# tatsuya-ogawa/GaussianSplattingMlx

Hardware: AMD Instinct MI355X
Metric: train views/sec (full step: fwd + L1/DSSIM loss + bwd + Adam + densify/prune at the reference cadence), Lego 800x800 300k Gaussians (higher is better)
Workload: dtype f32

## Files before the change

gaussiansplattingmlx_amd/_lib.py:

```python
from __future__ import annotations

import ctypes as C
import os

HERE = os.path.dirname(os.path.abspath(__file__))
LIB_PATH = os.environ.get("GSPLAT_LIB", os.path.join(HERE, "libgsplat_hip.so"))

GS_OK = 0
STATUS = {1: "GS_ERR_INVALID_ARG", 2: "GS_ERR_SIZE_MISMATCH", 3: "GS_ERR_WORKSPACE_OVERFLOW", 4: "GS_ERR_HIP",
          5: "GS_ERR_NO_FORWARD", 6: "GS_ERR_NO_DEVICE", 7: "GS_ERR_IO", 8: "GS_ERR_COMM", 9: "GS_ERR_REPLICA_MISMATCH"}
GS_ERR_REPLICA_MISMATCH = 9


class GsplatError(RuntimeError):
    def __init__(self, code, msg):
        super().__init__(f"{STATUS.get(code, code)}: {msg}")
        self.code = code


class gs_camera(C.Structure):
    _fields_ = [("view", C.c_float * 16), ("proj", C.c_float * 16), ("cam_center", C.c_float * 3),
                ("fov_x", C.c_float), ("fov_y", C.c_float), ("focal_x", C.c_float), ("focal_y", C.c_float)]


# ... 88 lines not shown
    "gs_ply_pack_rows": (C.c_int, [_vp, C.c_int, C.c_int] + [_vp] * 7),
    "gs_set_block_work_buffer": (C.c_int, [_vp, _vp]),
    "gs_view_hint_words": (C.c_int, [_vp, C.POINTER(C.c_int)]),
    "gs_set_view_hints": (C.c_int, [_vp, _vp, C.c_int]),
    "gs_set_depth_cuts": (C.c_int, [_vp, C.c_int]),
    "gs_clear_depth_cuts": (C.c_int, [_vp, _vp, C.c_int]),
    "gs_forward_missed": (C.c_int, [_vp, C.POINTER(C.c_int)]),
    "gs_cut_stats": (C.c_int, [_vp, C.POINTER(C.c_uint32)]),
    "gs_set_grad_norm_accum": (C.c_int, [_vp, _vp]),
    "gs_block_count": (C.c_int, [_vp, _vp]),
    "gs_copy_block_work": (C.c_int, [_vp, _vp]),
    "gs_dist_topk": (C.c_int, [_vp, C.c_int, C.c_int, C.c_int, C.c_int, _vp, _vp]),
    "gs_sh_grad_from_views_adam": (C.c_int, [_vp, C.c_int, C.c_int, C.c_int] + [_vp] * 8 + [C.c_longlong] + [C.c_float] * 6),
    "gs_loss_target_cache_floats": (C.c_int, [_vp, C.POINTER(C.c_longlong)]),
    "gs_set_loss_target_cache": (C.c_int, [_vp, _vp, C.c_int]),
    "gs_set_loss_mask": (C.c_int, [_vp, _vp]),
    "gs_loss_forward_backward": (C.c_int, [_vp] + [_vp] * 5 + [C.c_float, C.c_float] + [_vp] * 3),
    "gs_depth_loss": (C.c_int, [_vp, C.POINTER(gs_depth_loss_params)] + [_vp] * 7),
    "gs_depth_normalize": (C.c_int, [_vp, C.c_longlong, _vp, _vp, C.c_float, _vp]),
    "gs_adam_step": (C.c_int, [_vp, C.c_longlong] + [_vp] * 4 + [C.c_int, _vp, _vp] + [C.c_float] * 4),
    "gs_profile_enable": (C.c_int, [_vp, C.c_uint]),
    "gs_profile_read": (C.c_int, [_vp, _vp, _vp]),
    "gs_copy_last_contrib": (C.c_int, [_vp, _vp]),
    "gs_last_stats": (C.c_int, [_vp, C.POINTER(C.c_uint32)]),
    "gs_ctx_set_tuning": (C.c_int, [_vp, C.c_int, C.c_longlong]),
    "gs_copy_overflow_flag": (C.c_int, [_vp, _vp]),
    "gs_set_update_gate": (C.c_int, [_vp, _vp]),
    "gs_set_overflow_rider": (C.c_int, [_vp, _vp]),
    "gs_set_pose_correction": (C.c_int, [_vp, _vp, _vp]),
    "gs_set_exposure": (C.c_int, [_vp, _vp, _vp]),
    "gs_apply_exposure": (C.c_int, [_vp, C.c_longlong, _vp, _vp, _vp]),
    "gs_set_bilateral_grid": (C.c_int, [_vp, _vp, _vp, C.c_int, C.c_int, C.c_int, C.c_float]),
    "gs_apply_bilateral_grid": (C.c_int, [_vp, C.c_int, C.c_int, _vp, C.c_int, C.c_int, C.c_int, _vp, _vp]),
    "gs_set_antialiasing": (C.c_int, [_vp, C.c_int]),
    "gs_set_background": (C.c_int, [_vp, _vp]),
    "gs_get_background": (C.c_int, [_vp, _vp]),
    "gs_composite_target": (C.c_int, [_vp, C.c_longlong, _vp, _vp, _vp, _vp]),
    "gs_set_absgrad": (C.c_int, [_vp, C.c_int]),
    "gs_get_absgrad": (C.c_int, [_vp, C.c_int, _vp]),
    "gs_set_sparse_adam": (C.c_int, [_vp, C.c_int]),
    "gs_get_visibility": (C.c_int, [_vp, C.c_int, _vp]),
    "gs_adam_step_visible": (C.c_int, [_vp, C.c_longlong] + [_vp] * 4 + [C.c_int, _vp, _vp, _vp] + [C.c_float] * 4 + [C.c_int, _vp]),
    "gs_set_filter3d_cameras": (C.c_int, [_vp, C.c_int, _vp]),
    "gs_compute_filter3d": (C.c_int, [_vp, C.c_int, _vp, _vp]),
    "gs_set_filter3d": (C.c_int, [_vp, _vp]),
    "gs_filter3d_bake": (C.c_int, [_vp, C.c_int] + [_vp] * 5),
# ... 14 lines not shown

_lib = None


def load():
    global _lib
    if _lib is not None:
        return _lib
    if not os.path.exists(LIB_PATH):
        raise ImportError(f"{LIB_PATH} is missing: run `python -m gaussiansplattingmlx_amd.build` "
                          "(or __graft_entry__.build()). There is no CPU fallback.")
    import torch
    lib = C.CDLL(LIB_PATH)
    for name, (res, args) in _SIGS.items():
        fn = getattr(lib, name)
        fn.restype = res
        fn.argtypes = args
    _lib = lib
    return lib


TUNE_FWD_WAVES_PER_SIMD, TUNE_BWD_WAVES_PER_CU, TUNE_FWD_QUADRANTS, TUNE_OP_FWD_PPL, TUNE_OP_BWD_PPL, \
    TUNE_FWD_TRACE_BUFFER, TUNE_DEPTH_GRADIENT, TUNE_WIDE_TILE_SORT, TUNE_HOST_OVERFLOW_ERRORS, TUNE_SPLITTER_DEPTH_SORT, \
    TUNE_COLOUR_RIDERS, TUNE_FWD_QUEUES, TUNE_FWD_FOUR_WAVES, TUNE_FWD_FOLD_TEST_SCALE, TUNE_POISON_CHECKPOINTS, TUNE_RENDER_ONLY, TUNE_FWD_PAIR, TUNE_FWD_SLOW_SLOT, TUNE_TRIM_RECTS = range(19)


def exported_symbols():
    return list(_SIGS)


def make_camera(view, proj, camCenter, fovX, fovY, focalX, focalY) -> gs_camera:
    import numpy as np
    cam = gs_camera()
    v = np.asarray(view, dtype=np.float32).reshape(16)
    p = np.asarray(proj, dtype=np.float32).reshape(16)
    cc = np.asarray(camCenter, dtype=np.float32).reshape(3)
    for i in range(16):
        cam.view[i] = float(v[i])
        cam.proj[i] = float(p[i])
    for i in range(3):
        cam.cam_center[i] = float(cc[i])
    cam.fov_x, cam.fov_y, cam.focal_x, cam.focal_y = float(fovX), float(fovY), float(focalX), float(focalY)
    return cam
```

gaussiansplattingmlx_amd/csrc/api.hip:

```cpp
#include <math.h>
#include <stdlib.h>
#include <stdio.h>
#include <string.h>

#include "gs_ctx.h"
#include <vector>

using namespace gs;

namespace {

int fail(gs_ctx* c, int code, const std::string& msg)
{
    if (c) c->err = msg;
    return code;
}

template <class T>
int dev_alloc(gs_ctx* c, T** p, size_t count)
{
    *p = nullptr;
    if (count == 0) count = 1;
    GS_HIP_CHECK(c, hipMalloc((void**)p, count * sizeof(T)));
    c->ws_bytes += count * sizeof(T);
// ... 820 lines not shown
    if (c->fwd.cutsActive && !c->fwd.missChecked) GS_HIP_CHECK(c, hipEventSynchronize(c->fwdDone));
    c->fwd.missed = false;
    c->fwd.bwdPrepared = false;
    c->fwd.arenaOverflow = false;
    c->fwd.cutStore = c->cutStore;
    c->fwd.cutsActive = c->cutStore != nullptr && c->allowCuts && N > 0;
    c->fwd.missChecked = !c->fwd.cutsActive;
    if (c->fwd.cutsActive) c->missHost[0] = 0;
    const CamParams cp = make_cam(cam, c->W, c->H);
    if (c->poseDelta) {
        const long long need = pose_partials_floats(N);
        if (need > c->posePartialsCap) {
            GS_HIP_CHECK(c, hipStreamSynchronize(c->stream));
            dev_free(c->posePartials);
            c->posePartialsCap = 0;
            if (const int arc = dev_alloc(c, &c->posePartials, (size_t)need)) return arc;
            c->posePartialsCap = need;
        }
        if (const int prc = launch_pose_camera(c, cp, c->poseDelta)) return prc;
    }
    c->segBaseWanted = c->fast16 && N > 0;
    c->segBaseDone = false;
    c->fwdPairNow = c->fast16 && blend_forward_v2_pair_decide(c);
    int rc = bin_with_capacity(c, N, reserved, !c->fast16, [&]() {
        return launch_projection_fused_forward(c, N, K, xyz, features_dc, features_rest, scales, rotation, opacity, cp,
                                               radii);
    });
    c->segBaseWanted = false;
    if (rc) { c->rider.on = false; return rc; }
    if (c->rider.on && c->rider.next < c->rider.total) {
        GsStageTimer t(c, GS_STAGE_PROJ_FWD, true);
        if ((rc = launch_colour_rest(c))) return rc;
    }
    c->rider.on = false;
    {
        GsStageTimer t(c, GS_STAGE_BLEND_FWD);
        rc = c->fast16 ? launch_blend_forward_v2(c, out_color, out_depth, out_alpha)
                       : launch_blend_forward(c, c->bg, out_color, out_depth, out_alpha, c->lastContrib);
        if (rc) return rc;
    }
    if (c->fwd.cutsActive) GS_HIP_CHECK(c, hipEventRecord(c->fwdDone, c->stream));
    c->fwd.valid = true;
    c->absgradN = -1;
    c->fwd.blendBackwardDone = false;
    c->fwd.consumed = false;
    c->fwd.blockWork = c->blockWork;
// ... 689 lines not shown
    case GS_TUNE_WIDE_TILE_SORT:
        c->wideTileSort = value != 0; return GS_OK;
    case GS_TUNE_DEPTH_GRADIENT:
        c->depthGradient = value != 0; return GS_OK;
    case GS_TUNE_HOST_OVERFLOW_ERRORS:
        c->hostOverflowErrors = value != 0; return GS_OK;
    case GS_TUNE_SPLITTER_DEPTH_SORT:
        c->splitterSort = value < 0 ? 0 : (value > 2 ? 2 : (int)value); c->haveSplitters = false; return GS_OK;
    case GS_TUNE_COLOUR_RIDERS:
        c->colourRiders = (int)value; return GS_OK;
    case GS_TUNE_FWD_FOLD_TEST_SCALE:
        if (value < 1 || value > 1000) return fail(c, GS_ERR_INVALID_ARG, "gs_ctx_set_tuning: fold test scale is in permille, 1..1000");
        c->fwdFoldScale = (float)value / 1000.0f; return GS_OK;
    case GS_TUNE_POISON_CHECKPOINTS:
        c->poisonCheckpoints = value != 0; return GS_OK;
    case GS_TUNE_RENDER_ONLY:
        c->renderOnly = value != 0; return GS_OK;
    case GS_TUNE_FWD_SLOW_SLOT:
        if (value < 1 || value > 16) return fail(c, GS_ERR_INVALID_ARG, "gs_ctx_set_tuning: the first slow wave slot must be 1..16 (16 = none)");
        c->fwdSlowSlot = (int)value; return GS_OK;
    case GS_TUNE_FWD_PAIR:
        if (value < -1 || value > 16) return fail(c, GS_ERR_INVALID_ARG, "gs_ctx_set_tuning: forward pair workgroups per CU must be -1 (by list depth), 0..16");
        c->fwdPair = (int)value; return GS_OK;
    case GS_TUNE_TRIM_RECTS:
        if (value < 0 || value > 2) return fail(c, GS_ERR_INVALID_ARG, "gs_ctx_set_tuning: trim rects is 0 (the reference's squares), 1 (cut by the ellipse's box) or 2 (and into four row groups)");
        c->trimRects = value != 0; c->rowGroups = value == 2; return GS_OK;
    case GS_TUNE_FWD_TRACE_BUFFER:
        c->fwdTrace = reinterpret_cast<unsigned long long*>((uintptr_t)value); return GS_OK;
    default:
        return fail(c, GS_ERR_INVALID_ARG, "gs_ctx_set_tuning: unknown knob");
    }
}

int gs_copy_overflow_flag(gs_ctx* c, uint32_t* out)
{
    if (!c || !out) return GS_ERR_INVALID_ARG;
    hipLaunchKernelGGL(copy_word_kernel, dim3(1), dim3(1), 0, c->stream, c->counters + GS_CNT_OVERFLOW, out);
    GS_HIP_CHECK(c, hipGetLastError());
    return GS_OK;
}

int gs_set_update_gate(gs_ctx* c, const uint32_t* gate)
{
    if (!c) return GS_ERR_INVALID_ARG;
    c->adamGate = gate ? gate : c->counters + GS_CNT_OVERFLOW;
    return GS_OK;
// ... 34 lines not shown
int gs_block_count(gs_ctx* c, int* n)
{
    if (!c || !n) return GS_ERR_INVALID_ARG;
    *n = c->numPixBlocks;
    return GS_OK;
}

int gs_copy_block_work(gs_ctx* c, uint32_t* out)
{
    if (!c || !out) return GS_ERR_INVALID_ARG;
    if (!c->fwd.valid) return fail(c, GS_ERR_NO_FORWARD, "gs_copy_block_work: no gs_render_forward on this context");
    if (!c->fast16) return fail(c, GS_ERR_INVALID_ARG, "gs_copy_block_work: only for tile sizes served by the fused kernels");
    GS_HIP_CHECK(c, hipMemcpyAsync(out, c->fwd.blockWork, sizeof(uint32_t) * (size_t)c->numPixBlocks, hipMemcpyDeviceToDevice,
                                   c->stream));
    return GS_OK;
}

int gs_copy_last_contrib(gs_ctx* c, uint32_t* out)
{
    if (!c || !out) return GS_ERR_INVALID_ARG;
    if (!c->fwd.valid) return fail(c, GS_ERR_NO_FORWARD, "gs_copy_last_contrib: no gs_render_forward on this context");
    GS_HIP_CHECK(c, hipMemcpyAsync(out, c->lastContrib, sizeof(uint32_t) * (size_t)c->W * c->H, hipMemcpyDeviceToDevice,
                                   c->stream));
    return GS_OK;
}

int gs_adam_step(gs_ctx* c, long long n, float* params, const float* grads, float* m, float* v, int nseg,
                 const long long* seg_end, const float* seg_lr, float beta1, float beta2, float eps, float grad_scale)
{
    if (!c) return GS_ERR_INVALID_ARG;
    if (n < 0 || nseg < 1 || nseg > 8 || !seg_end || !seg_lr) return fail(c, GS_ERR_INVALID_ARG, "gs_adam_step: bad segments");
    if (n > 0 && (!params || !grads || !m || !v)) return fail(c, GS_ERR_INVALID_ARG, "gs_adam_step: null buffer");
    if (((uintptr_t)params | (uintptr_t)grads | (uintptr_t)m | (uintptr_t)v) & 15)
        return fail(c, GS_ERR_INVALID_ARG, "gs_adam_step: arenas must be 16-byte aligned");
    long long prev = 0;
    for (int i = 0; i < nseg; i++) {
        if (seg_end[i] < prev || seg_end[i] > n) return fail(c, GS_ERR_INVALID_ARG, "gs_adam_step: segments not ascending");
        prev = seg_end[i];
    }
    if (prev != n) return fail(c, GS_ERR_SIZE_MISMATCH, "gs_adam_step: segments do not cover the arena");
    { const int orc = deferred_overflow(c); if (orc) return orc; }
    return launch_adam(c, n, params, grads, m, v, nseg, seg_end, seg_lr, beta1, beta2, eps, grad_scale);
}

int gs_adam_step_visible(gs_ctx* c, long long n, float* params, const float* grads, float* m, float* v, int nseg,
                         const long long* seg_end, const float* seg_lr, const int* seg_row_floats, float beta1, float beta2,
// ... 266 lines not shown
```

gaussiansplattingmlx_amd/csrc/blend_v2.hip:

```cpp
#include "gs_ctx.h"
#include "gs_bwd_prep.h"
#include "gs_cull.h"
#include "gs_wavesum.h"

namespace gs {

constexpr int BLK = 16;
constexpr uint32_t CKPT_POOL_MAX = 8;
static inline uint32_t ckpt_pool(uint32_t partSlots, uint32_t waves)
{
    const uint32_t perWave = partSlots / (waves / 8u + 1u);
    return perWave >= CKPT_POOL_MAX ? CKPT_POOL_MAX : (perWave < 1u ? 1u : perWave);
}

struct Rec {
    float mx, my, c00, c01, c10, c11, r, g, b, op, depth;
};

#ifndef GS_FWD_PREFETCH
#define GS_FWD_PREFETCH 1
#endif

typedef float f4 __attribute__((ext_vector_type(4)));
typedef float f2 __attribute__((ext_vector_type(2)));
// ... 488 lines not shown

        V2P_BARRIER();
        for (uint32_t c0 = 0; c0 < count; c0 += 64) {
            const uint32_t cur = (c0 >> 6) & 1u;
            const f4* sl = sg[cur];
            const uint32_t n = __builtin_amdgcn_readfirstlane(*(volatile uint32_t*)&sN[cur]);
            br += cr; bgr += cg; bb += cb; cr = 0.f; cg = 0.f; cb = 0.f;
            if (DEPTH) { bd += dd; dd = 0.f; }
            if (statePlanes != 0 && c0 != 0 && (c0 % SEG) == 0) save_state(c0);
            bool live = true;
            for (uint32_t j = 0; j < n; j += 4) {
                Pre p0, p1, p2, p3;
                pre(sl, j, p0); pre(sl, j + 1, p1); pre(sl, j + 2, p2); pre(sl, j + 3, p3);
                post(p0); post(p1); post(p2); post(p3);
                if (!any_live()) { live = false; break; }
            }
            if (live) {
                if (T >= 1e-4f) nc = min(c0 + 64u, count);
                live = any_live();
            }
            if (!live && lane == 0) sStop = 1u;
            V2P_BARRIER();
            if (*(volatile uint32_t*)&sStop) break;
        }
        V2P_BARRIER();
        if (bRaw != 0xFFFFFFFFu) {
            if (cutStore && any_live() && lane == 0 && cutStore[tile] != 0u) hostWords[0] = 1u;
            if (in) {
                const size_t pix = (size_t)y * W + x;
                float bg0, bg1, bg2;
                gs_bg_terms(bgc, T, bg0, bg1, bg2);
                outColor[3 * pix] = (br + cr) + bg0; outColor[3 * pix + 1] = (bgr + cg) + bg1; outColor[3 * pix + 2] = (bb + cb) + bg2;
                if (DEPTH) outDepth[pix] = bd + dd;
                outAlpha[pix] = 1.0f - T; lastContrib[pix] = nc; finalT[pix] = T;
            }
            uint32_t m = in ? nc : 0u;
#pragma unroll
            for (int d = 32; d >= 1; d >>= 1) m = max(m, (uint32_t)__shfl_xor((int)m, d, 64));
            if (lane == 0 && m) atomicMax(&blockWork[b], m);
        }
    }
}
#undef V2P_BARRIER

#define GS_V2W_WGS 5
template <int SEG, bool DEPTH>
// ... 504 lines not shown
                const uint32_t src = (0x6a4b98331ull >> ((q - 2) * 4)) & 15u;
                v = (DEPTH || q != 10) ? part[j][src] : 0.0f;
                if (q < 6) v *= -0.5f;
            }
            if (v != 0.0f) atomicAdd(&gradAcc16[(size_t)(idx[i0 + j] & idxMask) * 16 + (ABSGRAD && q >= 11 ? q + 1 : q)], v);
        }
        __builtin_amdgcn_s_waitcnt(0xc07f);
        __builtin_amdgcn_wave_barrier();
    }
}

constexpr int SEGLEN = GS_SEG_LEN;
bool blend_forward_v2_wide(const gs_ctx* c)
{
    if (c->fwdTrace || !c->fwdQuadrants) return false;
    return c->fwdWide == 1 || (c->fwdWide < 0 && c->numPixBlocks * 4 <= c->numCUs * 4 * c->fwdWavesPerSimd);
}
bool blend_forward_v2_pair_decide(const gs_ctx* c)
{
    if (c->fwdTrace || !c->fwdQuadrants || blend_forward_v2_wide(c)) return false;
    if (c->fwdPair >= 0) return c->fwdPair != 0;
    const unsigned long long lastM = c->missHost ? c->missHost[8] : 0u;
    return c->numPixBlocks > 0 && lastM / (unsigned long long)c->numPixBlocks >= 4500ull;
}
bool blend_forward_v2_pair(const gs_ctx* c)
{
    return c->fwdPairNow;
}
int blend_forward_v2_grid(const gs_ctx* c)
{
    const int fwdItems = c->numPixBlocks * 4;
    const int fwdGrid = blend_forward_v2_wide(c) ? c->numCUs * GS_V2W_WGS
                        : blend_forward_v2_pair(c) ? c->numCUs * (c->fwdPair > 1 ? c->fwdPair : GS_V2P_WGS)
                                                   : c->numCUs * 4 * c->fwdWavesPerSimd;
    return fwdGrid > fwdItems ? fwdItems : fwdGrid;
}

void fill_seg_base(gs_ctx* c, SegBaseArgs& a)
{
    a.nBlocks = c->numPixBlocks; a.blocksX = c->blocksX; a.tileW = c->tileW; a.tileH = c->tileH; a.gridW = c->gridW;
    a.tileRanges = c->tileRanges; a.tileTotal = nullptr;
    a.segBase = c->segBase; a.blockWork = c->blockWork; a.counters = c->counters; a.workHint = c->workHint;
    a.blockOrder = c->blockOrder; a.queueStart = (uint32_t)blend_forward_v2_grid(c); a.fwdQueue = c->fwdQueue; a.nq = c->fwdQueues; a.spatial = c->fwdSpatial;
}

int launch_blend_forward_v2(gs_ctx* c, float* outColor, float* outDepth, float* outAlpha)
// ... 23 lines not shown
        c->fwd.qslotStatic = ownW * (uint32_t)grid * 4u;
        const uint32_t partW = (qcap - c->fwd.qslotStatic) / 8u;
        auto kw = outDepth ? blend_fwd_v2w_kernel<SEGLEN, true> : blend_fwd_v2w_kernel<SEGLEN, false>;
        hipLaunchKernelGGL(kw, dim3(grid), dim3(256), 0, c->stream, c->W, c->H, c->tileW,
                           c->tileH, c->gridW, blocksX, nItems, c->bg, reinterpret_cast<const float4*>(c->packed12),
                           c->sortedRaw, c->idxMask, c->tileRanges, c->segBase, (uint32_t)c->segCap, c->renderOnly ? 0 : c->fwd.statePlanes, outColor, outDepth,
                           outAlpha, c->lastContrib, c->finalT, c->segState, c->segSlot, qcap, ownW, partW, ckpt_pool(partW, (uint32_t)grid * 4u), c->blockWork, c->counters, c->fwdQueue,
                           (uint32_t)c->fwdQueues, c->blockOrder, cuts, c->missDev, c->fwdFoldScale, c->virt);
        GS_HIP_CHECK(c, hipGetLastError());
        if (c->renderOnly) c->fwd.statePlanes = 0;
        return GS_OK;
    }
    if (blend_forward_v2_pair(c)) {
        auto kp = outDepth ? blend_fwd_v2p_kernel<SEGLEN, true> : blend_fwd_v2p_kernel<SEGLEN, false>;
        hipLaunchKernelGGL(kp, dim3(grid), dim3(128), 0, c->stream, c->W, c->H, c->tileW,
                           c->tileH, c->gridW, blocksX, nItems, c->bg, reinterpret_cast<const float4*>(c->packed12),
                           c->sortedRaw, c->idxMask, c->tileRanges, c->segBase, (uint32_t)c->segCap, c->renderOnly ? 0 : c->fwd.statePlanes, outColor, outDepth,
                           outAlpha, c->lastContrib, c->finalT, c->segState, c->segSlot, qcap, own, partSlots, ckpt_pool(partSlots, (uint32_t)grid), c->blockWork, c->counters, c->fwdQueue, (uint32_t)c->fwdQueues, c->blockOrder,
                           cuts, c->missDev, c->virt);
        GS_HIP_CHECK(c, hipGetLastError());
        if (c->renderOnly) c->fwd.statePlanes = 0;
        return GS_OK;
    }
    auto kern = outDepth ? blend_fwd_v2q_kernel<SEGLEN, true> : blend_fwd_v2q_kernel<SEGLEN, false>;
    hipLaunchKernelGGL(kern, dim3(grid / 4), dim3(256), 0, c->stream, c->W, c->H, c->tileW,
                       c->tileH, c->gridW, blocksX, nItems, c->bg, reinterpret_cast<const float4*>(c->packed12),
                       c->sortedRaw, c->idxMask, c->tileRanges, c->segBase, (uint32_t)c->segCap, c->renderOnly ? 0 : c->fwd.statePlanes, outColor, outDepth,
                       outAlpha, c->lastContrib, c->finalT, c->segState, c->segSlot, qcap, own, partSlots, ckpt_pool(partSlots, (uint32_t)grid), c->blockWork, c->counters, c->fwdQueue, (uint32_t)c->fwdQueues, c->blockOrder,
                       c->fwdTrace, cuts, c->missDev, (uint32_t)c->fwdSlowSlot, c->virt);
    GS_HIP_CHECK(c, hipGetLastError());
    if (c->renderOnly) c->fwd.statePlanes = 0;
    return GS_OK;
}

void fill_bwd_prep(gs_ctx* c, int N, uint32_t queueStart, BwdPrepArgs& p)
{
    p.nBlocks = c->numPixBlocks;
    p.blockWork = c->fwd.blockWork;
    p.itemBlock = c->itemBlock;
    p.itemRow = c->itemRow;
    p.segBase = c->segBase;
    p.itemCap = (uint32_t)c->itemCap;
    p.counters = c->counters;
    p.queueStart = queueStart;
    p.bwdQueue = c->bwdQueue;
    p.clearBuf = reinterpret_cast<float4*>(c->gradAcc16);
// ... 43 lines not shown
```

gaussiansplattingmlx_amd/csrc/gs_ctx.h:

```cpp
#pragma once
#include <hip/hip_runtime.h>
#include <stdint.h>

#include <string>
#include <vector>

#include "../../include/gsplat.h"
#include "gs_math.h"

enum {
    GS_CNT_M = 0,
    GS_CNT_OVERFLOW = 1,
    GS_CNT_MREQ = 2,
    GS_CNT_B = 3,
    GS_CNT_NVIS = 4,
    GS_CNT_CONTRIB_LO = 5,
    GS_CNT_CONTRIB_HI = 6,
    GS_CNT_ITEMS = 9,
    GS_CNT_QUEUE = 10,
    GS_CNT_QUEUE_FWD = 11,
    GS_CNT_CUT_DROPPED = 12,
    GS_CNT_QSLOTS = 16,
    GS_CNT_COUNT = 24
};
// ... 60 lines not shown
struct GsVirtGeom {
    int nbx = 0, nby = 0;
    int tw = 0, th = 0;
};
__device__ __forceinline__ void gs_block_pixels(const GsVirtGeom& g, int bx, int by, int W, int H, int& X0, int& Y0, int& XL, int& YL)
{
    if (g.nbx == 0) { X0 = bx * 16; Y0 = by * 16; XL = W; YL = H; return; }
    const int tx = bx / g.nbx, ix = bx - tx * g.nbx, ty = by / g.nby, iy = by - ty * g.nby;
    X0 = tx * g.tw + ix * 16; Y0 = ty * g.th + iy * 16;
    XL = min(W, min(X0 + 16, (tx + 1) * g.tw)); YL = min(H, min(Y0 + 16, (ty + 1) * g.th));
}
constexpr int GS_F3D_CAM_FLOATS = 16;
constexpr int GS_CUT_SUPER = 4;
struct GsCutCoarse {
    const uint32_t* superCut = nullptr;
    int superW = 0;
    uint32_t* dropPerBlock = nullptr;
};
struct GsRealGeom {
    int tileW = 16, tileH = 16, gridW = 0, gridH = 0, T = 0, tileBits = 1;
    bool fast16 = false;
};

struct gs_ctx {
    int device = 0;
    GsDp* dp = nullptr;
    hipStream_t stream = nullptr;
    hipStream_t own_stream = nullptr;
    int W = 0, H = 0, tileW = 16, tileH = 16, gridW = 0, gridH = 0, T = 0, degree = 0, whiteBg = 0;
    int tileBits = 1;
    GsBackground bg;
    bool fast16 = false;
    GsVirtGeom virt;
    GsRealGeom real;
    bool binIsBlockLists = false;
    int blocksX = 0, blocksY = 0;
    std::string err;

    int capN = 0;
    long long capM = 0;
    bool pairsReserved = false;
    bool reserving = false;
    size_t ws_bytes = 0;

    float* packed12 = nullptr;
    float* gradAcc16 = nullptr;
// ... 86 lines not shown
    uint32_t* segBase = nullptr;
    float* segState = nullptr;
    uint32_t* segSlot = nullptr;
    long long segCap = 0;
    long long qslotCap = 0;
    long long qslotWanted = 0;
    bool arenaRegrowPending = false;
    uint32_t* itemBlock = nullptr;
    uint32_t* itemRow = nullptr;
    long long itemCap = 0;
    float* finalT = nullptr;
    int numCUs = 256;
    int numPixBlocks = 0;
    int opBlocks = 0;
    int fwdWavesPerSimd = 4, bwdWavesPerCu = 16;
    int fwdQuadrants = 1;
    int scatterThreads = 0;
    int lsdThreads = 0;
    int fwdWide = -1;
    float fwdFoldScale = 1.0f;
    int fwdSlowSlot = 3;
    int fwdPair = -1;
    bool fwdPairNow = false;
    bool trimRects = true;
    bool rowGroups = true;
    int renderOnly = 0;
    int poisonCheckpoints = 0;
    int rankSort = 1;
    int fwdSpatial = 0;
    int fwdQueues = 8;
    int opFwdPpl = 1, opBwdPpl = 1;
    bool segBaseWanted = false;
    bool segBaseDone = false;
    int wideTileSort = 1;
    int hostOverflowErrors = 1;
    int depthGradient = 1;
    unsigned long long* fwdTrace = nullptr;
    const uint32_t* adamGate = nullptr;
    float* overflowRider = nullptr;
    long long ccBlockFloats = 0;
    int ccBlockCount = 0;
    uint32_t* gatheredGateOut = nullptr;
    uint32_t* gateSeen = nullptr;
    uint32_t* lastContrib = nullptr;
    float* lossPartials = nullptr;
    float* lossTargetCache = nullptr;
// ... 166 lines not shown
int launch_bin_prep(gs_ctx* c, int N, const float* rectMin, const float* rectMax, const float* radii,
                    const float* depths);
int launch_binning(gs_ctx* c, int N, bool wantPlain);
int ensure_plain_sorted(gs_ctx* c);
int launch_tile_counts(gs_ctx* c);
int launch_cut_super(gs_ctx* c, const uint32_t* cuts);
int cut_super_width(const gs_ctx* c);
int launch_build_packed_tile_indices(gs_ctx* c, uint32_t B, int32_t* out);

int launch_blend_forward(gs_ctx* c, const GsBackground& bg, float* outColor, float* outDepth, float* outAlpha, uint32_t* lastContrib);
int launch_blend_backward(gs_ctx* c, const GsBackground& bg, int N, const float* cotColor, const float* cotDepth, const float* cotAlpha,
                          const float* outAlpha, const uint32_t* lastContrib);
int launch_gradacc_to_packed11(gs_ctx* c, int N, float* gradPacked11);

int launch_blend_contrib(gs_ctx* c, float* maxW, float* sumW);
int launch_contrib_actions(gs_ctx* c, int N, const float* score, float threshold, int* actions, int* outputCounts);

int launch_blend_forward_v2(gs_ctx* c, float* outColor, float* outDepth, float* outAlpha);
int launch_blend_backward_v2(gs_ctx* c, int N, const float* cotColor, const float* cotDepth, const float* cotAlpha,
                             const float* outColor, const float* outDepth, const float* outAlpha, bool absgrad = false);
int blend_backward_v2_grid(const gs_ctx* c);
int blend_forward_v2_grid(const gs_ctx* c);
bool blend_forward_v2_pair_decide(const gs_ctx* c);

int launch_ssim_forward(gs_ctx* c, int H, int W, int C, int K, const float* img1, const float* img2,
                        const float* window, float* ssim, float* mu1, float* mu2, float* s1, float* s2, float* s12);
int launch_ssim_backward(gs_ctx* c, int H, int W, int C, int K, const float* gradOut, float gradOutConst,
                         const float* img1, const float* img2, const float* window, const float* mu1,
                         const float* mu2, const float* s1, const float* s2, const float* s12, float* g1, float* g2,
                         float l1Weight);
int launch_loss(gs_ctx* c, const float* render, const float* target, const float* renderDepth,
                const float* targetDepth, const unsigned char* depthMask, float lambdaDssim, float lambdaDepth,
                float* lossOut, float* cotColor, float* cotDepth);

int launch_accum_grad_norm(gs_ctx* c, int N, const float* xyzGrad, const float* accumIn, float* accumOut);
int launch_absgrad_accum(gs_ctx* c, int N, const uint32_t* gate, float* accum);
int launch_absgrad_copy(gs_ctx* c, int N, float* out);
int launch_classify(gs_ctx* c, int N, const float* gradAccum, float denom, const float* scales, int scaleStride,
                    const float* opacity, float gradThreshold, float maxScale, float minOpacity, int allowDensify,
                    int* actions, int* outputCounts);
int launch_densify_offsets(gs_ctx* c, int N, const int* actions, const int* outputCounts, int* offsets,
                           long long stats[5]);
int launch_build_densify_map(gs_ctx* c, int N, const int* actions, const int* offsets, int total, int* gather,
                             int* noiseMode);
int launch_densify_gather(gs_ctx* c, int total, int K, const float* xyz, const float* fdc, const float* frest,
                          const float* scales, const float* rot, const float* opacity, const int* gather,
// ... 45 lines not shown
```

gaussiansplattingmlx_amd/renderer.py:

```python
from __future__ import annotations

import ctypes as C
import math
import os
from collections import OrderedDict, namedtuple

import numpy as np
import torch

from . import _lib, loss_mask
from ._lib import GsplatError

TILE_SIZE_H_W = namedtuple("TILE_SIZE_H_W", ["w", "h"])
RenderResult = namedtuple("RenderResult", ["render", "depth", "alpha", "visiility_filter", "radii"])


def _p(t):
    return None if t is None else C.c_void_p(t.data_ptr())


def _f32(t, device):
    if isinstance(t, torch.Tensor):
        return t.to(device=device, dtype=torch.float32).contiguous()
    return torch.as_tensor(np.ascontiguousarray(t, dtype=np.float32), device=device)
# ... 97 lines not shown
        return _f32(t, self.device)

    def _measure(self, name, body):
        return self.profiler.measure(name, body) if self.profiler is not None else body()

    def _empty(self, *shape, dtype=torch.float32):
        return torch.empty(shape, dtype=dtype, device=self.device)

    def reserve(self, max_gaussians: int, max_pairs: int):
        self._check(self.lib.gs_ctx_reserve(self.ctx, int(max_gaussians), int(max_pairs)))
        self.reserved = (int(max_gaussians), int(max_pairs))

    def sync(self):
        self._check(self.lib.gs_sync(self.ctx))

    _TUNING = dict(fwd_waves_per_simd=_lib.TUNE_FWD_WAVES_PER_SIMD, bwd_waves_per_cu=_lib.TUNE_BWD_WAVES_PER_CU,
                   fwd_quadrants=_lib.TUNE_FWD_QUADRANTS, op_fwd_ppl=_lib.TUNE_OP_FWD_PPL,
                   op_bwd_ppl=_lib.TUNE_OP_BWD_PPL, fwd_trace_buffer=_lib.TUNE_FWD_TRACE_BUFFER,
                   depth_gradient=_lib.TUNE_DEPTH_GRADIENT, wide_tile_sort=_lib.TUNE_WIDE_TILE_SORT,
                   host_overflow_errors=_lib.TUNE_HOST_OVERFLOW_ERRORS, splitter_depth_sort=_lib.TUNE_SPLITTER_DEPTH_SORT,
                   colour_riders=_lib.TUNE_COLOUR_RIDERS, fwd_queues=_lib.TUNE_FWD_QUEUES, fwd_four_waves=_lib.TUNE_FWD_FOUR_WAVES,
                   fwd_fold_test_scale=_lib.TUNE_FWD_FOLD_TEST_SCALE, poison_checkpoints=_lib.TUNE_POISON_CHECKPOINTS,
                   render_only=_lib.TUNE_RENDER_ONLY, fwd_pair=_lib.TUNE_FWD_PAIR, fwd_slow_slot=_lib.TUNE_FWD_SLOW_SLOT,
                   trim_rects=_lib.TUNE_TRIM_RECTS)
    _TUNING_DEFAULTS = dict(fwd_waves_per_simd=4, bwd_waves_per_cu=16, fwd_quadrants=1, op_fwd_ppl=1, op_bwd_ppl=1,
                            fwd_trace_buffer=0, depth_gradient=1, wide_tile_sort=1, host_overflow_errors=1, splitter_depth_sort=1,
                            colour_riders=1, fwd_queues=8, fwd_four_waves=-1, fwd_fold_test_scale=1000, poison_checkpoints=0, render_only=0, fwd_pair=-1, fwd_slow_slot=3, trim_rects=2)

    def setTuning(self, **knobs):
        for k, v in knobs.items():
            self._check(self.lib.gs_ctx_set_tuning(self.ctx, self._TUNING[k], int(v)))
            self._tuning_now = {**getattr(self, "_tuning_now", {}), k: int(v)}

    def getTuning(self, knob: str) -> int:
        return getattr(self, "_tuning_now", {}).get(knob, self._TUNING_DEFAULTS[knob])

    def colourRidersActive(self, N: int, K: int = 25) -> bool:
        if K != 25 or self.getTuning("colour_riders") != 1 or ((self.TILE_SIZE.w % 16 or self.TILE_SIZE.h % 16) and not self.blockLists):
            return False
        split = self.getTuning("splitter_depth_sort")
        return bool(split) and N > 16384 and (N <= 160 * 4096 or (split >= 2 and N <= 1024 * 4096))

    def stats(self):
        s = (C.c_uint32 * 8)()
        self._check(self.lib.gs_last_stats(self.ctx, s))
        return dict(N_visible=s[0], M=s[1], max_tile_list=s[2], overflow=s[5], capN=s[6], capM=s[7])

    @staticmethod
    def _camera(viewMatrix, projMatrix, cameraCenter, fovX, fovY, focalX, focalY):
        g = lambda a: a.detach().cpu().numpy() if isinstance(a, torch.Tensor) else a
# ... 240 lines not shown

    def renderChecked(self, params: dict, camera, want_radii: bool = False, viewKey=None, wantDepth: bool = True):
        res = self.renderForward(params, camera, want_radii, viewKey, wantDepth=wantDepth)
        if self.forwardMissed():
            res = self.renderForward(params, camera, want_radii, viewKey, depthCuts=False, wantDepth=wantDepth)
        return res

    @property
    def blockLists(self) -> bool:
        return (self.TILE_SIZE.w % 16 != 0 or self.TILE_SIZE.h % 16 != 0) and os.environ.get("GSPLAT_BLOCK_LISTS", "1") != "0"

    def blockWork(self):
        n = C.c_int()
        self._check(self.lib.gs_block_count(self.ctx, C.byref(n)))
        out = self._empty(n.value, dtype=torch.int32)
        self._check(self.lib.gs_copy_block_work(self.ctx, _p(out)))
        return out

    def lastContrib(self):
        out = self._empty(self.H, self.W, dtype=torch.int32)
        self._check(self.lib.gs_copy_last_contrib(self.ctx, _p(out)))
        return out

    STAGES = ("proj_fwd", "bin", "blend_fwd", "loss", "blend_bwd", "proj_bwd", "adam")

    def profile(self, stages=True):
        if stages is True:
            mask = (1 << len(self.STAGES)) - 1
        elif not stages:
            mask = 0
        else:
            mask = sum(1 << self.STAGES.index(s) for s in stages)
        self._check(self.lib.gs_profile_enable(self.ctx, mask))

    def profileRead(self):
        ms, calls = (C.c_float * 8)(), (C.c_int * 8)()
        self._check(self.lib.gs_profile_read(self.ctx, ms, calls))
        return {n: (ms[i], calls[i]) for i, n in enumerate(self.STAGES)}

    def renderBackward(self, cotColor, cotDepth=None, cotAlpha=None, out: dict | None = None):
        p = self._fused["params"]
        g = out or {k: torch.empty_like(v) for k, v in p.items()}
        cotColor = self._t(cotColor)
        cotDepth = None if cotDepth is None else self._t(cotDepth)
        cotAlpha = None if cotAlpha is None else self._t(cotAlpha)
        self._cuts_renewed()
# ... 533 lines not shown
```

include/gsplat.h:

```cpp
#ifndef GSPLAT_H
#define GSPLAT_H

#include <stddef.h>
#include <stdint.h>

#ifdef __cplusplus
extern "C" {
#endif

#define GSPLAT_ABI_VERSION 6

typedef enum gs_status {
    GS_OK = 0,
    GS_ERR_INVALID_ARG = 1,
    GS_ERR_SIZE_MISMATCH = 2,
    GS_ERR_WORKSPACE_OVERFLOW = 3,
    GS_ERR_HIP = 4,
    GS_ERR_NO_FORWARD = 5,
    GS_ERR_NO_DEVICE = 6,
    GS_ERR_IO = 7,
    GS_ERR_COMM = 8,
    GS_ERR_REPLICA_MISMATCH = 9
} gs_status;

// ... 307 lines not shown
int gs_set_update_gate(gs_ctx* ctx, const uint32_t* gate );
int gs_set_overflow_rider(gs_ctx* ctx, float* dst );
int gs_set_gathered_gate(gs_ctx* ctx, long long block_floats, int count, uint32_t* reduced_out );
int gs_set_gate_seen(gs_ctx* ctx, uint32_t* seen );

typedef enum gs_tuning {
    GS_TUNE_FWD_WAVES_PER_SIMD = 0,
    GS_TUNE_BWD_WAVES_PER_CU = 1,
    GS_TUNE_FWD_QUADRANTS = 2,
    GS_TUNE_OP_FWD_PPL = 3,
    GS_TUNE_OP_BWD_PPL = 4,
    GS_TUNE_FWD_TRACE_BUFFER = 5,
    GS_TUNE_WIDE_TILE_SORT = 7,
    GS_TUNE_HOST_OVERFLOW_ERRORS = 8,
    GS_TUNE_SPLITTER_DEPTH_SORT = 9,
    GS_TUNE_COLOUR_RIDERS = 10,
    GS_TUNE_FWD_QUEUES = 11,
    GS_TUNE_FWD_FOUR_WAVES = 12,
    GS_TUNE_FWD_FOLD_TEST_SCALE = 13,
    GS_TUNE_RENDER_ONLY = 15,
    GS_TUNE_FWD_PAIR = 16,
    GS_TUNE_FWD_SLOW_SLOT = 17,
    GS_TUNE_TRIM_RECTS = 18,
    GS_TUNE_POISON_CHECKPOINTS = 14,
    GS_TUNE_DEPTH_GRADIENT = 6
} gs_tuning;
int gs_ctx_set_tuning(gs_ctx* ctx, int knob, long long value);

int gs_block_count(gs_ctx* ctx, int* n);
int gs_copy_block_work(gs_ctx* ctx, uint32_t* out);
int gs_copy_last_contrib(gs_ctx* ctx, uint32_t* out);

#ifdef __cplusplus
}
#endif
#endif
```

Before: 653.0.

## Add block-staged forward blend kernel sharing record loads across four waves

Adds a new forward blend kernel in which the four waves of a 256-thread workgroup take turns loading 64-record chunks of a 16x16 block's list. Each chunk is culled per 8x8 quadrant into double-buffered shared memory, replacing independent per-wave gathers. Early termination is coordinated through shared stop masks, and checkpoint state saving is kept. The kernel is selected by default unless the pair-kernel rule fires, which adds workgroup barriers per chunk and more shared-memory use in exchange for fewer redundant global loads. A finalT copy API is also added.

```diff
diff --git a/gaussiansplattingmlx_amd/_lib.py b/gaussiansplattingmlx_amd/_lib.py
--- a/gaussiansplattingmlx_amd/_lib.py
+++ b/gaussiansplattingmlx_amd/_lib.py
@@ -134,6 +134,7 @@
     "gs_profile_enable": (C.c_int, [_vp, C.c_uint]),
     "gs_profile_read": (C.c_int, [_vp, _vp, _vp]),
     "gs_copy_last_contrib": (C.c_int, [_vp, _vp]),
+    "gs_copy_final_t": (C.c_int, [_vp, _vp]),
     "gs_last_stats": (C.c_int, [_vp, C.POINTER(C.c_uint32)]),
     "gs_ctx_set_tuning": (C.c_int, [_vp, C.c_int, C.c_longlong]),
     "gs_copy_overflow_flag": (C.c_int, [_vp, _vp]),
@@ -194,7 +195,7 @@
 
 TUNE_FWD_WAVES_PER_SIMD, TUNE_BWD_WAVES_PER_CU, TUNE_FWD_QUADRANTS, TUNE_OP_FWD_PPL, TUNE_OP_BWD_PPL, \
     TUNE_FWD_TRACE_BUFFER, TUNE_DEPTH_GRADIENT, TUNE_WIDE_TILE_SORT, TUNE_HOST_OVERFLOW_ERRORS, TUNE_SPLITTER_DEPTH_SORT, \
-    TUNE_COLOUR_RIDERS, TUNE_FWD_QUEUES, TUNE_FWD_FOUR_WAVES, TUNE_FWD_FOLD_TEST_SCALE, TUNE_POISON_CHECKPOINTS, TUNE_RENDER_ONLY, TUNE_FWD_PAIR, TUNE_FWD_SLOW_SLOT, TUNE_TRIM_RECTS = range(19)
+    TUNE_COLOUR_RIDERS, TUNE_FWD_QUEUES, TUNE_FWD_FOUR_WAVES, TUNE_FWD_FOLD_TEST_SCALE, TUNE_POISON_CHECKPOINTS, TUNE_RENDER_ONLY, TUNE_FWD_PAIR, TUNE_FWD_SLOW_SLOT, TUNE_TRIM_RECTS, TUNE_FWD_BLOCK = range(20)
 
 
 def exported_symbols():
diff --git a/gaussiansplattingmlx_amd/csrc/api.hip b/gaussiansplattingmlx_amd/csrc/api.hip
--- a/gaussiansplattingmlx_amd/csrc/api.hip
+++ b/gaussiansplattingmlx_amd/csrc/api.hip
@@ -866,6 +866,9 @@
     c->segBaseWanted = c->fast16 && N > 0;
     c->segBaseDone = false;
     c->fwdPairNow = c->fast16 && blend_forward_v2_pair_decide(c);
+    c->fwdBlockNow = c->fast16 && blend_forward_v2_block_decide(c);
+    if (c->fwdBlockNow && c->fwdBlock < 0 && c->fwdPairNow) c->fwdBlockNow = false;
+    if (c->fwdBlockNow) c->fwdPairNow = false;
     int rc = bin_with_capacity(c, N, reserved, !c->fast16, [&]() {
         return launch_projection_fused_forward(c, N, K, xyz, features_dc, features_rest, scales, rotation, opacity, cp,
                                                radii);
@@ -1601,6 +1604,9 @@
     case GS_TUNE_FWD_PAIR:
         if (value < -1 || value > 16) return fail(c, GS_ERR_INVALID_ARG, "gs_ctx_set_tuning: forward pair workgroups per CU must be -1 (by list depth), 0..16");
         c->fwdPair = (int)value; return GS_OK;
+    case GS_TUNE_FWD_BLOCK:
+        if (value < -1 || value > 1) return fail(c, GS_ERR_INVALID_ARG, "gs_ctx_set_tuning: forward block staging is -1 (by rule), 0 or 1");
+        c->fwdBlock = (int)value; return GS_OK;
     case GS_TUNE_TRIM_RECTS:
         if (value < 0 || value > 2) return fail(c, GS_ERR_INVALID_ARG, "gs_ctx_set_tuning: trim rects is 0 (the reference's squares), 1 (cut by the ellipse's box) or 2 (and into four row groups)");
         c->trimRects = value != 0; c->rowGroups = value == 2; return GS_OK;
@@ -1681,6 +1687,14 @@
     if (!c->fwd.valid) return fail(c, GS_ERR_NO_FORWARD, "gs_copy_last_contrib: no gs_render_forward on this context");
     GS_HIP_CHECK(c, hipMemcpyAsync(out, c->lastContrib, sizeof(uint32_t) * (size_t)c->W * c->H, hipMemcpyDeviceToDevice,
                                    c->stream));
+    return GS_OK;
+}
+
+int gs_copy_final_t(gs_ctx* c, float* out)
+{
+    if (!c || !out) return GS_ERR_INVALID_ARG;
+    if (!c->fwd.valid) return fail(c, GS_ERR_NO_FORWARD, "gs_copy_final_t: no gs_render_forward on this context");
+    GS_HIP_CHECK(c, hipMemcpyAsync(out, c->finalT, sizeof(float) * (size_t)c->W * c->H, hipMemcpyDeviceToDevice, c->stream));
     return GS_OK;
 }
 
diff --git a/gaussiansplattingmlx_amd/csrc/blend_v2.hip b/gaussiansplattingmlx_amd/csrc/blend_v2.hip
--- a/gaussiansplattingmlx_amd/csrc/blend_v2.hip
+++ b/gaussiansplattingmlx_amd/csrc/blend_v2.hip
@@ -534,6 +534,220 @@
             if (!live && lane == 0) sStop = 1u;
             V2P_BARRIER();
             if (*(volatile uint32_t*)&sStop) break;
+        }
+        V2P_BARRIER();
+        if (bRaw != 0xFFFFFFFFu) {
+            if (cutStore && any_live() && lane == 0 && cutStore[tile] != 0u) hostWords[0] = 1u;
+            if (in) {
+                const size_t pix = (size_t)y * W + x;
+                float bg0, bg1, bg2;
+                gs_bg_terms(bgc, T, bg0, bg1, bg2);
+                outColor[3 * pix] = (br + cr) + bg0; outColor[3 * pix + 1] = (bgr + cg) + bg1; outColor[3 * pix + 2] = (bb + cb) + bg2;
+                if (DEPTH) outDepth[pix] = bd + dd;
+                outAlpha[pix] = 1.0f - T; lastContrib[pix] = nc; finalT[pix] = T;
+            }
+            uint32_t m = in ? nc : 0u;
+#pragma unroll
+            for (int d = 32; d >= 1; d >>= 1) m = max(m, (uint32_t)__shfl_xor((int)m, d, 64));
+            if (lane == 0 && m) atomicMax(&blockWork[b], m);
+        }
+    }
+}
+
+template <int SEG, bool DEPTH>
+__global__ __launch_bounds__(256) void blend_fwd_v2b_kernel(
+    int W, int H, int tileW, int tileH, int gridW, int blocksX, int nItems, GsBackground bgc,
+    const float4* __restrict__ rec12, const uint32_t* __restrict__ sortedIdx, uint32_t idxMask,
+    const uint32_t* __restrict__ tileRanges, const uint32_t* __restrict__ segBase, uint32_t segCap, int statePlanes,
+    float* __restrict__ outColor, float* __restrict__ outDepth,
+    float* __restrict__ outAlpha, uint32_t* __restrict__ lastContrib, float* __restrict__ finalT,
+    float* __restrict__ segState, uint32_t* __restrict__ segSlot, uint32_t qslotCap, uint32_t qslotOwn, uint32_t qslotPart, uint32_t ckptPool,
+    uint32_t* __restrict__ blockWork, uint32_t* __restrict__ counters, uint32_t* __restrict__ fwdQueue, uint32_t nq,
+    const uint32_t* __restrict__ blockOrder, const uint32_t* __restrict__ cutStore, uint32_t* __restrict__ hostWords, GsVirtGeom vg)
+{
+    static_assert(SEG % 64 == 0, "segment length must be a multiple of the 64-record chunk");
+    __shared__ f4 sg[4][2][192];
+    __shared__ uint32_t sN[2][4];
+    __shared__ uint32_t sItem;
+    __shared__ uint32_t sStop[2];
+    const int lane = threadIdx.x & 63;
+    const uint32_t wv = (uint32_t)__builtin_amdgcn_readfirstlane((int)(threadIdx.x >> 6));
+    const uint32_t nWaves = gridDim.x * 4u;
+    const uint32_t dw = blockIdx.x * 4u + wv;
+    uint32_t poolNext = dw * qslotOwn, poolEnd = poolNext + qslotOwn;
+    const uint32_t part = blockIdx.x & 7u;
+    uint32_t partsEmpty = 0;
+    const uint32_t xcd = blockIdx.x % nq, row = blockIdx.x / nq;
+    const uint32_t nPos = nq * ((((uint32_t)nItems >> 2) + nq - 1u) / nq);
+    const uint32_t staticRows = gridDim.x / nq;
+    uint32_t dead = 0;
+    for (bool first = true;; first = false) {
+        if (wv == 0) {
+            uint32_t pos = 0xFFFFFFFFu;
+            if (first && row < staticRows) pos = nq * row + xcd;
+            else {
+                for (uint32_t t = 0; t < nq && pos == 0xFFFFFFFFu; t++) {
+                    const uint32_t y = (xcd + t) % nq;
+                    if ((dead >> y) & 1u) continue;
+                    uint32_t k = 0;
+                    if (lane == 0) k = atomicAdd(&fwdQueue[y * 32u], 4u);
+                    k = __builtin_amdgcn_readfirstlane(k);
+                    const uint32_t p = nq * (staticRows + (k >> 2)) + y;
+                    if (p < nPos) pos = p;
+                    else dead |= 1u << y;
+                }
+            }
+            if (lane == 0) { sItem = pos; sStop[0] = 0u; sStop[1] = 0u; }
+        }
+        __syncthreads();
+        const uint32_t pos = __builtin_amdgcn_readfirstlane(*(volatile uint32_t*)&sItem);
+        if (pos >= nPos) {
+            __syncthreads();
+            if (first) continue;
+            break;
+        }
+        const uint32_t bRaw = __builtin_amdgcn_readfirstlane(blockOrder[pos]);
+        const int b = (int)bRaw;
+        const int h = (int)((wv >> 1) & 1u), k = (int)(wv & 1u);
+        uint32_t start = 0, count = 0, sbase = 0;
+        int tile = 0, X0 = 0, Y0 = 0, XL = 0, YL = 0;
+        if (bRaw != 0xFFFFFFFFu) {
+            const int by = b / blocksX, bx = b - by * blocksX;
+            tile = ((by * BLK) / tileH) * gridW + (bx * BLK) / tileW;
+            start = __builtin_amdgcn_readfirstlane(tileRanges[2 * tile]);
+            const uint32_t end = __builtin_amdgcn_readfirstlane(tileRanges[2 * tile + 1]);
+            count = end > start ? end - start : 0u;
+            sbase = __builtin_amdgcn_readfirstlane(segBase[b]);
+            gs_block_pixels(vg, bx, by, W, H, X0, Y0, XL, YL);
+        }
+        const int x = X0 + k * 8 + (lane & 7), y = Y0 + h * 8 + (lane >> 3);
+        const bool in = bRaw != 0xFFFFFFFFu && x < XL && y < YL;
+        const float px = (float)x, py = (float)y;
+        const uint32_t* __restrict__ idx = sortedIdx + start;
+
+        auto stage_block = [&](uint32_t sl, const RecV& v, uint32_t c0, uint32_t stopped) {
+            const bool inList = c0 + (uint32_t)lane < count;
+            const f4 tagged = (f4){v.c.x, v.c.y, v.c.z, __uint_as_float(c0 + (uint32_t)lane + 1u)};
+            const f4 z = (f4){0.f, 0.f, 0.f, 0.f};
+            const f4 padTag = (f4){0.f, 0.f, 0.f, __uint_as_float(min(c0 + 64u, count))};
+#pragma unroll
+            for (uint32_t q = 0; q < 4u; q++) {
+                if ((stopped >> q) & 1u) continue;
+                const float qx0 = (float)(X0 + (int)(q & 1u) * 8), qx1 = qx0 + 7.0f;
+                const float qy0 = (float)(Y0 + (int)(q >> 1) * 8), qy1 = qy0 + 7.0f;
+                const float qmin = rect_min_q(v.a.z, v.a.w, v.b.x, v.b.y, qx0 - v.a.x, qx1 - v.a.x, qy0 - v.a.y, qy1 - v.a.y);
+                const bool keep = inList && !(qmin > CULL_QMIN);
+                const unsigned long long m = __ballot(keep);
+                const uint32_t ps = (uint32_t)__popcll(m & ((1ull << lane) - 1ull));
+                f4* slot = sg[q][sl];
+                if (keep) { slot[ps * 3] = v.a; slot[ps * 3 + 1] = v.b; slot[ps * 3 + 2] = tagged; }
+                const uint32_t n = (uint32_t)__popcll(m), n4 = (n + 3u) & ~3u;
+                if ((uint32_t)lane < n4 - n) { slot[(n + lane) * 3] = z; slot[(n + lane) * 3 + 1] = z; slot[(n + lane) * 3 + 2] = padTag; }
+                if (lane == 0) sN[sl][q] = n4;
+            }
+        };
+        RecV nxt;
+        nxt.a = nxt.b = nxt.c = (f4){0.f, 0.f, 0.f, 0.f};
+        uint32_t gNext = 0xFFFFFFFFu;
+        if (64u * wv < count) {
+            gNext = load_chunk_index(idx, idxMask, 64u * wv + 256u, count, lane);
+            nxt = load_chunk(rec12, idx, idxMask, 64u * wv, count, lane);
+        }
+        auto stage_turn = [&](uint32_t c0, uint32_t stopped) {
+            stage_block((c0 >> 6) & 1u, nxt, c0, stopped);
+            if (c0 + 256u < count) {
+                nxt = gather_chunk(rec12, gNext);
+                gNext = load_chunk_index(idx, idxMask, c0 + 512u, count, lane);
+            }
+        };
+
+        float T = in ? 1.0f : 0.0f;
+        float cr = 0.f, cg = 0.f, cb = 0.f, dd = 0.f;
+        float br = 0.f, bgr = 0.f, bb = 0.f, bd = 0.f;
+        uint32_t nc = 0;
+        auto save_state = [&](uint32_t i) {
+            if (poolNext == poolEnd) {
+                poolNext = qslotCap;
+                for (uint32_t t = 0; t < 8u && poolNext == qslotCap; t++) {
+                    const uint32_t yy = (part + t) & 7u;
+                    if ((partsEmpty >> yy) & 1u) continue;
+                    uint32_t base = 0;
+                    if (lane == 0) base = atomicAdd(&counters[GS_CNT_QSLOTS + yy], ckptPool);
+                    base = __builtin_amdgcn_readfirstlane(base);
+                    if (base + ckptPool <= qslotPart) poolNext = nWaves * qslotOwn + yy * qslotPart + base;
+                    else {
+                        partsEmpty |= 1u << yy;
+                        if (lane == 0) atomicSub(&counters[GS_CNT_QSLOTS + yy], ckptPool);
+                    }
+                }
+                if (poolNext == qslotCap && partsEmpty == 0xFFu && lane == 0) atomicAdd(&counters[GS_CNT_QSLOTS + part], ckptPool);
+                poolEnd = poolNext + ckptPool;
+            }
+            const uint32_t phys = poolNext++;
+            const uint32_t vslot = sbase + i / SEG - 1;
+            if (phys < qslotCap && vslot < segCap) {
+                if (lane == 0) segSlot[(size_t)vslot * 4 + (h * 2 + k)] = phys;
+                float* st = segState + (size_t)phys * (statePlanes * 64) + lane;
+                if (T >= 1e-4f) {
+                    st[0] = T; st[64] = br; st[128] = bgr; st[192] = bb;
+                    if (DEPTH && statePlanes == 5) st[256] = bd;
+                }
+            } else if (lane == 0) {
+                counters[GS_CNT_OVERFLOW] = 1u;
+                hostWords[4] = 2u;
+            }
+        };
+        struct Pre {
+            float aclamp, r, g, b, depth;
+            uint32_t ncv;
+        };
+        auto pre = [&](const f4* sl, uint32_t j, Pre& o) {
+            const Rec s = unpack(sl[j * 3], sl[j * 3 + 1], sl[j * 3 + 2]);
+            const float dx = px - s.mx, dy = py - s.my;
+            const float dxdy = dx * dy, dx2 = dx * dx, dy2 = dy * dy;
+            const float q = ((dx2 * s.c00 + dy2 * s.c11) + dxdy * s.c01) + dxdy * s.c10;
+            o.aclamp = fminf(gauss_alpha_raw(q, s.op), 0.99f);
+            o.r = s.r; o.g = s.g; o.b = s.b; o.depth = s.depth;
+            o.ncv = __float_as_uint(sl[j * 3 + 2].w);
+        };
+        auto post = [&](const Pre& o) {
+            const bool a = T >= 1e-4f;
+            nc = a ? o.ncv : nc;
+            const float alpha = a ? o.aclamp : 0.0f;
+            const float w = T * alpha;
+            cr = fmaf(w, o.r, cr); cg = fmaf(w, o.g, cg); cb = fmaf(w, o.b, cb); if (DEPTH) dd = fmaf(w, o.depth, dd);
+            T = T * (1.0f - alpha);
+        };
+        auto any_live = [&]() { return __any(T >= 1e-4f); };
+
+        if (!any_live() && lane == 0) atomicOr(&sStop[1], 1u << wv);
+        if (wv == 0 && count > 0) stage_turn(0, 0u);
+        V2P_BARRIER();
+        uint32_t stopped = __builtin_amdgcn_readfirstlane(*(volatile uint32_t*)&sStop[1]);
+        for (uint32_t c0 = 0; c0 < count && stopped != 15u; c0 += 64) {
+            const uint32_t cur = (c0 >> 6) & 1u;
+            if (c0 + 64 < count && (((c0 >> 6) + 1u) & 3u) == wv) stage_turn(c0 + 64, stopped);
+            if (!((stopped >> wv) & 1u)) {
+                const f4* sl = sg[wv][cur];
+                const uint32_t n = __builtin_amdgcn_readfirstlane(*(volatile uint32_t*)&sN[cur][wv]);
+                br += cr; bgr += cg; bb += cb; cr = 0.f; cg = 0.f; cb = 0.f;
+                if (DEPTH) { bd += dd; dd = 0.f; }
+                if (statePlanes != 0 && c0 != 0 && (c0 % SEG) == 0) save_state(c0);
+                bool live = true;
+                for (uint32_t j = 0; j < n; j += 4) {
+                    Pre p0, p1, p2, p3;
+                    pre(sl, j, p0); pre(sl, j + 1, p1); pre(sl, j + 2, p2); pre(sl, j + 3, p3);
+                    post(p0); post(p1); post(p2); post(p3);
+                    if (!any_live()) { live = false; break; }
+                }
+                if (live) {
+                    if (T >= 1e-4f) nc = min(c0 + 64u, count);
+                    live = any_live();
+                }
+                if (!live && lane == 0) atomicOr(&sStop[cur], 1u << wv);
+            }
+            V2P_BARRIER();
+            stopped |= __builtin_amdgcn_readfirstlane(*(volatile uint32_t*)&sStop[cur]);
         }
         V2P_BARRIER();
         if (bRaw != 0xFFFFFFFFu) {
@@ -1084,6 +1298,11 @@
     if (c->fwdPair >= 0) return c->fwdPair != 0;
     const unsigned long long lastM = c->missHost ? c->missHost[8] : 0u;
     return c->numPixBlocks > 0 && lastM / (unsigned long long)c->numPixBlocks >= 4500ull;
+}
+bool blend_forward_v2_block_decide(const gs_ctx* c)
+{
+    if (c->fwdTrace || !c->fwdQuadrants || blend_forward_v2_wide(c)) return false;
+    return c->fwdBlock != 0;
 }
 bool blend_forward_v2_pair(const gs_ctx* c)
 {
@@ -1153,6 +1372,17 @@
         if (c->renderOnly) c->fwd.statePlanes = 0;
         return GS_OK;
     }
+    if (c->fwdBlockNow) {
+        auto kb = outDepth ? blend_fwd_v2b_kernel<SEGLEN, true> : blend_fwd_v2b_kernel<SEGLEN, false>;
+        hipLaunchKernelGGL(kb, dim3(grid / 4), dim3(256), 0, c->stream, c->W, c->H, c->tileW,
+                           c->tileH, c->gridW, blocksX, nItems, c->bg, reinterpret_cast<const float4*>(c->packed12),
+                           c->sortedRaw, c->idxMask, c->tileRanges, c->segBase, (uint32_t)c->segCap, c->renderOnly ? 0 : c->fwd.statePlanes, outColor, outDepth,
+                           outAlpha, c->lastContrib, c->finalT, c->segState, c->segSlot, qcap, own, partSlots, ckpt_pool(partSlots, (uint32_t)grid), c->blockWork, c->counters, c->fwdQueue, (uint32_t)c->fwdQueues, c->blockOrder,
+                           cuts, c->missDev, c->virt);
+        GS_HIP_CHECK(c, hipGetLastError());
+        if (c->renderOnly) c->fwd.statePlanes = 0;
+        return GS_OK;
+    }
     auto kern = outDepth ? blend_fwd_v2q_kernel<SEGLEN, true> : blend_fwd_v2q_kernel<SEGLEN, false>;
     hipLaunchKernelGGL(kern, dim3(grid / 4), dim3(256), 0, c->stream, c->W, c->H, c->tileW,
                        c->tileH, c->gridW, blocksX, nItems, c->bg, reinterpret_cast<const float4*>(c->packed12),
diff --git a/gaussiansplattingmlx_amd/csrc/gs_ctx.h b/gaussiansplattingmlx_amd/csrc/gs_ctx.h
--- a/gaussiansplattingmlx_amd/csrc/gs_ctx.h
+++ b/gaussiansplattingmlx_amd/csrc/gs_ctx.h
@@ -106,6 +106,9 @@
     bool fast16 = false;
 };
 
+#ifndef GS_FWD_BLOCK_DEFAULT
+#define GS_FWD_BLOCK_DEFAULT (-1)
+#endif
 struct gs_ctx {
     int device = 0;
     GsDp* dp = nullptr;
@@ -238,6 +241,8 @@
     int fwdSlowSlot = 3;
     int fwdPair = -1;
     bool fwdPairNow = false;
+    int fwdBlock = GS_FWD_BLOCK_DEFAULT;
+    bool fwdBlockNow = false;
     bool trimRects = true;
     bool rowGroups = true;
     int renderOnly = 0;
@@ -450,6 +455,7 @@
 int blend_backward_v2_grid(const gs_ctx* c);
 int blend_forward_v2_grid(const gs_ctx* c);
 bool blend_forward_v2_pair_decide(const gs_ctx* c);
+bool blend_forward_v2_block_decide(const gs_ctx* c);
 
 int launch_ssim_forward(gs_ctx* c, int H, int W, int C, int K, const float* img1, const float* img2,
                         const float* window, float* ssim, float* mu1, float* mu2, float* s1, float* s2, float* s12);
diff --git a/gaussiansplattingmlx_amd/renderer.py b/gaussiansplattingmlx_amd/renderer.py
--- a/gaussiansplattingmlx_amd/renderer.py
+++ b/gaussiansplattingmlx_amd/renderer.py
@@ -143,10 +143,10 @@
                    colour_riders=_lib.TUNE_COLOUR_RIDERS, fwd_queues=_lib.TUNE_FWD_QUEUES, fwd_four_waves=_lib.TUNE_FWD_FOUR_WAVES,
                    fwd_fold_test_scale=_lib.TUNE_FWD_FOLD_TEST_SCALE, poison_checkpoints=_lib.TUNE_POISON_CHECKPOINTS,
                    render_only=_lib.TUNE_RENDER_ONLY, fwd_pair=_lib.TUNE_FWD_PAIR, fwd_slow_slot=_lib.TUNE_FWD_SLOW_SLOT,
-                   trim_rects=_lib.TUNE_TRIM_RECTS)
+                   trim_rects=_lib.TUNE_TRIM_RECTS, fwd_block=_lib.TUNE_FWD_BLOCK)
     _TUNING_DEFAULTS = dict(fwd_waves_per_simd=4, bwd_waves_per_cu=16, fwd_quadrants=1, op_fwd_ppl=1, op_bwd_ppl=1,
                             fwd_trace_buffer=0, depth_gradient=1, wide_tile_sort=1, host_overflow_errors=1, splitter_depth_sort=1,
-                            colour_riders=1, fwd_queues=8, fwd_four_waves=-1, fwd_fold_test_scale=1000, poison_checkpoints=0, render_only=0, fwd_pair=-1, fwd_slow_slot=3, trim_rects=2)
+                            colour_riders=1, fwd_queues=8, fwd_four_waves=-1, fwd_fold_test_scale=1000, poison_checkpoints=0, render_only=0, fwd_pair=-1, fwd_slow_slot=3, trim_rects=2, fwd_block=-1)
 
     def setTuning(self, **knobs):
         for k, v in knobs.items():
@@ -433,6 +433,11 @@
         self._check(self.lib.gs_copy_last_contrib(self.ctx, _p(out)))
         return out
 
+    def finalT(self):
+        out = self._empty(self.H, self.W, dtype=torch.float32)
+        self._check(self.lib.gs_copy_final_t(self.ctx, _p(out)))
+        return out
+
     STAGES = ("proj_fwd", "bin", "blend_fwd", "loss", "blend_bwd", "proj_bwd", "adam")
 
     def profile(self, stages=True):
diff --git a/include/gsplat.h b/include/gsplat.h
--- a/include/gsplat.h
+++ b/include/gsplat.h
@@ -353,6 +353,7 @@
     GS_TUNE_FWD_PAIR = 16,
     GS_TUNE_FWD_SLOW_SLOT = 17,
     GS_TUNE_TRIM_RECTS = 18,
+    GS_TUNE_FWD_BLOCK = 19,
     GS_TUNE_POISON_CHECKPOINTS = 14,
     GS_TUNE_DEPTH_GRADIENT = 6
 } gs_tuning;
@@ -361,6 +362,7 @@
 int gs_block_count(gs_ctx* ctx, int* n);
 int gs_copy_block_work(gs_ctx* ctx, uint32_t* out);
 int gs_copy_last_contrib(gs_ctx* ctx, uint32_t* out);
+int gs_copy_final_t(gs_ctx* ctx, float* out);
 
 #ifdef __cplusplus
 }
```

Result: slower. 645.4 (-1.2%).
